# ZhicengShi/mclSTExp

Measured on AMD Instinct MI355X. Metric: training spots/sec (= steps/sec x global batch) at batch 128/GPU, 224px patches, 1000 genes, higher is better.
Workload: dtype bf16; 1 GPU; BASELINE configs[1]: train step, batch 128/GPU, 224x224 patches, 1000 genes, densenet121 image encoder; global_batch=128, parallelism=dp1, backbone_dtype=bf16, infonce=fused, infonce_effective=exact (fused from 1024 pairs), hip_graphs=True, optimizer=Adam(lr=1e-4, wd=1e-3) incl. 2x(65536,G) tables

## Files before the change

### include/mclstexp_hip.h

```cpp
#ifndef MCLSTEXP_HIP_H
#define MCLSTEXP_HIP_H

#include <stddef.h>
#include <stdint.h>

#ifdef __cplusplus
extern "C" {
#endif

#define MCL_ABI_VERSION 13

#define MCL_OK 0
#define MCL_EINVAL (-1)
#define MCL_EUNSUPPORTED (-2)
#define MCL_EWORKSPACE (-3)

typedef void* mcl_stream_t;

int mcl_abi_version(void);
const char* mcl_error_string(int code);

#define MCL_EPI_GELU 1
#define MCL_EPI_GELU_BWD 2
#define MCL_EPI_ACCUM 4
// ... 211 lines not shown
int mcl_dense_bn1_fix(const void* x, int64_t ldx, void* gbuf, int64_t ldg, int64_t S, int32_t c0, int32_t nc,
                      const float* mean, const float* rstd, const float* kacc, mcl_stream_t stream);
int mcl_conv1x1_wrw_det(const void* dz, int64_t ldz, const void* a, int64_t lda, const float* gamma, const float* beta,
                        const float* mean, const float* rstd, float* workspace, float* dW, int32_t accumulate_w,
                        int64_t S, int32_t M, int32_t N, mcl_stream_t stream);

int64_t mcl_dense_conv3x3_bwd_workspace_floats(int64_t S);
int mcl_dense_conv3x3_bwd(const void* dy, int64_t lddy, int64_t S, int32_t H, int32_t W, const void* W2, const void* z,
                          const float* gamma, const float* beta, const float* mean, const float* rstd, float* workspace,
                          float* dgamma, float* dbeta, int32_t accumulate_params, void* g2, void* dz, mcl_stream_t stream);
int mcl_dense_conv3x3_bwd_fix(const void* dy, int64_t lddy, int64_t S, int32_t H, int32_t W, const void* W2, const void* z,
                              const float* gamma, const float* beta, const float* mean, const float* rstd, float* workspace,
                              float* dgamma, float* dbeta, int32_t accumulate_params, void* g2, void* dz, const void* xfix,
                              int64_t ldxf, const float* fmean, const float* frstd, const float* fk, void* dyc,
                              mcl_stream_t stream);

int mcl_avgpool2_nhwc_bf16(const void* x, void* y, int32_t N, int32_t H, int32_t W, int32_t C, int32_t backward,
                           mcl_stream_t stream);
int mcl_maxpool3s2_nhwc_bf16_fwd(const void* x, void* y, void* idx, int32_t N, int32_t H, int32_t W, int32_t C,
                                 mcl_stream_t stream);
int mcl_maxpool3s2_nhwc_bf16_bwd(const void* idx, const void* dy, void* dx, int32_t N, int32_t H, int32_t W, int32_t C,
                                 mcl_stream_t stream);
int mcl_maxpool3s2_nhwc_bf16_bwd_ld(const void* idx, const void* dy, int64_t lddy, void* dx, int32_t N, int32_t H, int32_t W,
                                    int32_t C, mcl_stream_t stream);

int mcl_bn_act_avgpool_fwd(const void* x, int64_t ldx, int32_t N, int32_t H, int32_t W, int32_t C, const float* gamma,
                           const float* beta, const float* mean, const float* rstd, void* y, int64_t ldy,
                           mcl_stream_t stream);
int mcl_bn_act_avgpool_bwd(const void* dp, int64_t lddp, const void* x, int64_t ldx, int32_t N, int32_t H, int32_t W,
                           int32_t C, const float* gamma, const float* beta, const float* mean, const float* rstd,
// ... 214 lines not shown
```

### mclstexp_amd/_lib.py

```python
from __future__ import annotations

import ctypes as C
import os
from typing import Optional

import torch

_HERE = os.path.dirname(os.path.abspath(__file__))
LIB_PATH = os.environ.get("MCL_LIB_PATH") or os.path.join(_HERE, "libmclstexp_hip.so")
ABI_VERSION = 13

_lib: Optional[C.CDLL] = None

c_f = C.c_float
c_d = C.c_double
c_i = C.c_int32
c_l = C.c_int64
c_p = C.c_void_p


class GemmArgs(C.Structure):
    _fields_ = [
        ("struct_size", C.c_uint32),
        ("M", c_i), ("N", c_i), ("K", c_i), ("batch", c_i),
# ... 117 lines not shown
    "mcl_bn_workspace_floats": [c_l, c_i, c_i],
    "mcl_bn_stats": [c_p, c_l, c_l, c_i, c_i, c_p, c_l, c_p, c_f, c_p, c_p, c_p, c_p],
    "mcl_bn_act_fwd": [c_p, c_l, c_l, c_i, c_i, c_p, c_p, c_p, c_p, c_i, c_p, c_l, c_p],
    "mcl_bn_act_bwd": [c_p, c_l, c_p, c_l, c_l, c_i, c_i, c_p, c_p, c_p, c_p, c_i, c_p, c_p, c_p, c_i, c_p, c_l, c_i, c_p],
    "mcl_dense_conv1x1_workspace_floats": [c_l],
    "mcl_dense_conv1x1_fwd": [c_p, c_l, c_l, c_i, c_p, c_p, c_p, c_p, c_p, c_p, c_l, c_p, c_f, c_p, c_p, c_p, c_p],
    "mcl_dense_conv3x3_workspace_floats": [c_l],
    "mcl_dense_bn1_bwd_workspace_floats": [c_l, c_i],
    "mcl_dense_conv3x3_bwd_workspace_floats": [c_l],
    "mcl_avgpool2_nhwc_bf16": [c_p, c_p, c_i, c_i, c_i, c_i, c_i, c_p],
    "mcl_maxpool3s2_nhwc_bf16_fwd": [c_p, c_p, c_p, c_i, c_i, c_i, c_i, c_p],
    "mcl_maxpool3s2_nhwc_bf16_bwd": [c_p, c_p, c_p, c_i, c_i, c_i, c_i, c_p],
    "mcl_dense_conv3x3_bwd": [c_p, c_l, c_l, c_i, c_i, c_p, c_p, c_p, c_p, c_p, c_p, c_p, c_p, c_p, c_i, c_p, c_p, c_p],
    "mcl_dense_conv3x3_bwd_fix": [c_p, c_l, c_l, c_i, c_i, c_p, c_p, c_p, c_p, c_p, c_p, c_p, c_p, c_p, c_i, c_p, c_p, c_p,
                                  c_l, c_p, c_p, c_p, c_p, c_p],
    "mcl_dense_bn1_bwd": [c_p, c_p, c_i, c_p, c_l, c_l, c_p, c_p, c_p, c_p, c_p, c_p, c_p, c_i, c_p, c_l, c_p],
    "mcl_dense_conv3x3_wrw_workspace_floats": [c_l],
    "mcl_dense_conv3x3_wrw_det": [c_p, c_l, c_p, c_l, c_i, c_i, c_p, c_p, c_p, c_p, c_p, c_p, c_i, c_p],
    "mcl_wrw_workspace_floats": [c_l, c_i, c_i],
    "mcl_dense_bn1_wrw": [c_p, c_p, c_i, c_p, c_l, c_l, c_p, c_p, c_p, c_p, c_p, c_p, c_i, c_p, c_p, c_i, c_p, c_p],
    "mcl_dense_bn1_dx_window": [c_p, c_p, c_i, c_i, c_i, c_p, c_l, c_l, c_p, c_p, c_p, c_p, c_p, c_p, c_l, c_p],
    "mcl_dense_bn1_dx_pair": [c_p, c_p, c_i, c_p, c_p, c_p, c_p, c_p, c_p, c_p, c_p, c_i, c_p, c_l, c_l, c_p, c_p, c_p, c_l, c_p],
    "mcl_dense_bn1_dx": [c_p, c_p, c_i, c_p, c_l, c_l, c_p, c_p, c_p, c_p, c_p, c_p, c_l, c_p],
    "mcl_dense_bn1_dx_sums": [c_p, c_p, c_i, c_p, c_l, c_l, c_p, c_p, c_p, c_p, c_p, c_p, c_p, c_i, c_p, c_i, c_p, c_l, c_p],
    "mcl_dense_bn1_fix": [c_p, c_l, c_p, c_l, c_l, c_i, c_i, c_p, c_p, c_p, c_p],
    "mcl_conv1x1_wrw_det": [c_p, c_l, c_p, c_l, c_p, c_p, c_p, c_p, c_p, c_p, c_i, c_l, c_i, c_i, c_p],
    "mcl_dense_conv3x3_fwd": [c_p, c_l, c_i, c_i, c_p, c_p, c_p, c_p, c_p, c_p, c_l, c_p, c_f, c_p, c_p, c_p, c_p],
    "mcl_accum_into_f32": [c_p, c_p, c_l, c_i, c_p],
    "mcl_adam_step": [c_p, c_p, c_p, c_p, c_l, c_d, c_d, c_d, c_d, c_d, c_d, c_d, c_p],
    "mcl_adam_table_step": [c_p, c_p, c_p, c_i, c_i, c_p, c_p, c_l, c_d, c_d, c_d, c_d, c_d, c_d, c_d, c_p],
# ... 161 lines not shown
```

### mclstexp_amd/csrc/dense_bwd.hip

```cpp
#include "common.h"
#include <stdlib.h>

namespace {

constexpr int TN = 128, TK = 128;

template <int MODE, int TMv>
__global__ __launch_bounds__(256, (TMv == 64 && MODE != 2 ? 3 : 2)) void bn1_bwd_kernel(const bf16_t* __restrict__ dz, const bf16_t* __restrict__ W1,
                                                         int K , int ldw ,
                                                         const bf16_t* __restrict__ x, long long ldx, long long S,
                                                         const float* __restrict__ gamma,
                                                         const float* __restrict__ beta,
                                                         const float* __restrict__ mean,
                                                         const float* __restrict__ rstd,
                                                         const float* __restrict__ coef ,
                                                         bf16_t* gbuf, long long ldg,
                                                         float2* __restrict__ partial , int nrt) {
  __shared__ __attribute__((aligned(16))) unsigned char lds[TK * 256 + TMv * 256 + 2048];
  const int tid = threadIdx.x, lane = tid & 63, wave = tid >> 6;
  const int h = lane >> 5, l31 = lane & 31;
  const int wm = wave >> 1, wn = wave & 1;
  const int n0 = blockIdx.y * TN;
  unsigned char* wt = lds;
  unsigned char* dzt = lds + TK * 256;
// ... 838 lines not shown
    const unsigned gw[4] = {gv.x, gv.y, gv.z, gv.w}, zw[4] = {zv.x, zv.y, zv.z, zv.w};
    unsigned o[4];
#pragma unroll
    for (int u = 0; u < 4; ++u) {
      const float g_lo = __uint_as_float(gw[u] << 16), g_hi = __uint_as_float(gw[u] & 0xFFFF0000u);
      const float z_lo = __uint_as_float(zw[u] << 16), z_hi = __uint_as_float(zw[u] & 0xFFFF0000u);
      const float d_lo = sc[2 * u] * (g_lo - c1[2 * u] - (z_lo - mu[2 * u]) * rs[2 * u] * c2[2 * u]);
      const float d_hi = sc[2 * u + 1] * (g_hi - c1[2 * u + 1] - (z_hi - mu[2 * u + 1]) * rs[2 * u + 1] * c2[2 * u + 1]);
      const f32x2 pv = {d_lo, d_hi};
      o[u] = __builtin_bit_cast(unsigned, __builtin_convertvector(pv, bf16x2_t));
    }
    *reinterpret_cast<uint4*>(dz + q * 8) = make_uint4(o[0], o[1], o[2], o[3]);
  }
}

}

extern "C" int64_t mcl_dense_bn1_bwd_workspace_floats(int64_t S, int32_t C) {
  if (S <= 0 || C <= 0) return -1;
  return ((S + 63) / 64) * 2 * (int64_t)C + 2 * (int64_t)C;
}

extern "C" int mcl_dense_bn1_bwd(const void* dz, const void* W1, int32_t C, const void* x, int64_t ldx, int64_t S,
                                 const float* gamma, const float* beta, const float* mean, const float* rstd,
                                 float* workspace, float* dgamma, float* dbeta, int32_t accumulate_params, void* gbuf,
                                 int64_t ldg, mcl_stream_t stream) {
  MCL_CLEAR_ERROR();
  if (!dz || !W1 || !x || !gamma || !beta || !mean || !rstd || !workspace || !dgamma || !dbeta || !gbuf || S <= 0 || C <= 0)
    return MCL_EINVAL;
  if ((C % 8) || (ldx % 8) || (ldg % 8) || (reinterpret_cast<uintptr_t>(dz) & 15u) ||
// ... 129 lines not shown
                     (const bf16_t*)x, (long long)ldx, (long long)S, mean, rstd, (bf16_t*)gbuf, (long long)ldg, nrt);
  MCL_CHECK_LAUNCH();
  return MCL_OK;
}

extern "C" int64_t mcl_dense_conv3x3_bwd_workspace_floats(int64_t S) {
  if (S <= 0) return -1;
  const int64_t flat = (S + T3B - 1) / T3B, rows = S / 32 + 8;
  return (flat > rows ? flat : rows) * 2 * (int64_t)C3I + 2 * (int64_t)C3I;
}

namespace {
int conv3x3_bwd_impl(const void* dy, int64_t lddy, int64_t S, int32_t H, int32_t W, const void* W2, const void* z,
                     const float* gamma, const float* beta, const float* mean, const float* rstd, float* workspace,
                     float* dgamma, float* dbeta, int32_t accumulate_params, void* g2, void* dz, const void* xfix,
                     int64_t ldxf, const float* fmean, const float* frstd, const float* fk, void* dyc, mcl_stream_t stream) {
  MCL_CLEAR_ERROR();
  if (!dy || !W2 || !z || !gamma || !beta || !mean || !rstd || !workspace || !dgamma || !dbeta || !g2 || !dz || S <= 0 ||
      H <= 0 || W <= 0)
    return MCL_EINVAL;
  if ((S % ((int64_t)H * W)) || S > 0x7fff0000LL || W > 150 || (lddy % 8) || lddy < C3O ||
      (reinterpret_cast<uintptr_t>(dy) & 15u) || (reinterpret_cast<uintptr_t>(z) & 15u) ||
      (reinterpret_cast<uintptr_t>(g2) & 15u) || (reinterpret_cast<uintptr_t>(dz) & 15u))
    return MCL_EUNSUPPORTED;
  if (xfix != nullptr) {
    if (!fmean || !frstd || !fk || !dyc) return MCL_EINVAL;
    if (bwd_rows_applicable(S, H, W) || (ldxf % 8) || (reinterpret_cast<uintptr_t>(xfix) & 15u) ||
        (reinterpret_cast<uintptr_t>(dyc) & 15u))
      return MCL_EUNSUPPORTED;
  }
  hipStream_t st = mcl_stream(stream);
  float2* part = reinterpret_cast<float2*>(workspace);
// ... 10 lines not shown
                       (const bf16_t*)dy, (long long)lddy, p.nimg, H, W, (const bf16_t*)W2, (const bf16_t*)z, gamma, beta,
                       mean, rstd, (bf16_t*)g2, part, p.nsu, p.rc, p.nchunk, p.nstrip);
    hipLaunchKernelGGL(bn1_bwd_finalize_kernel, dim3(C3I), dim3(256), 0, st, (const float2*)part, p.nsu, C3I,
                       (long long)S, dgamma, dbeta, coef, accumulate_params);
  } else {
    const int ntile = (int)((S + T3B - 1) / T3B);
    coef = workspace + (int64_t)ntile * 2 * C3I;
    const size_t lds_bytes = (size_t)T3B * 256 + (size_t)(T3B + 2 * W + 2) * 64 + 64;
    const int gcap = S >= 50000 ? 512 : 768;
    hipLaunchKernelGGL(conv3x3_bwd_kernel, dim3(ntile < gcap ? ntile : gcap), dim3(256), lds_bytes, st, (const bf16_t*)dy,
                       (long long)lddy, (long long)S, H, W, (const bf16_t*)W2, (const bf16_t*)z, gamma, beta, mean, rstd,
                       (bf16_t*)g2, part, ntile, (const bf16_t*)xfix, (long long)ldxf, fmean, frstd, fk, (bf16_t*)dyc);
    hipLaunchKernelGGL(bn1_bwd_finalize_kernel, dim3(C3I), dim3(256), 0, st, (const float2*)part, ntile, C3I,
                       (long long)S, dgamma, dbeta, coef, accumulate_params);
  }
  const long long n_chunks = S * (C3I / 8);
  long long blocks = (n_chunks + 255) / 256;
  if (blocks > 2048) blocks = 2048;
  hipLaunchKernelGGL(bn2_dz_kernel, dim3((unsigned)blocks), dim3(256), 0, st, (const bf16_t*)g2, (const bf16_t*)z,
                     n_chunks, gamma, mean, rstd, (const float*)coef, (bf16_t*)dz);
  MCL_CHECK_LAUNCH();
  return MCL_OK;
}
}

extern "C" int mcl_dense_conv3x3_bwd(const void* dy, int64_t lddy, int64_t S, int32_t H, int32_t W, const void* W2,
                                     const void* z, const float* gamma, const float* beta, const float* mean,
                                     const float* rstd, float* workspace, float* dgamma, float* dbeta,
                                     int32_t accumulate_params, void* g2, void* dz, mcl_stream_t stream) {
  return conv3x3_bwd_impl(dy, lddy, S, H, W, W2, z, gamma, beta, mean, rstd, workspace, dgamma, dbeta, accumulate_params, g2,
                          dz, nullptr, 0, nullptr, nullptr, nullptr, nullptr, stream);
}

extern "C" int mcl_dense_conv3x3_bwd_fix(const void* dy, int64_t lddy, int64_t S, int32_t H, int32_t W, const void* W2,
                                         const void* z, const float* gamma, const float* beta, const float* mean,
                                         const float* rstd, float* workspace, float* dgamma, float* dbeta,
                                         int32_t accumulate_params, void* g2, void* dz, const void* xfix, int64_t ldxf,
                                         const float* fmean, const float* frstd, const float* fk, void* dyc,
                                         mcl_stream_t stream) {
  if (!xfix) return MCL_EINVAL;
  return conv3x3_bwd_impl(dy, lddy, S, H, W, W2, z, gamma, beta, mean, rstd, workspace, dgamma, dbeta, accumulate_params, g2,
                          dz, xfix, ldxf, fmean, frstd, fk, dyc, stream);
}
```

### mclstexp_amd/densenet_fused.py

```python
from __future__ import annotations

import contextlib
import os
from typing import List, NamedTuple, Optional, Tuple

import torch
import torch.nn.functional as F
from torch import nn

from . import _lib
from ._lib import check

Tensor = torch.Tensor
CL = torch.channels_last
_ws_cache = {}

_fallbacks: dict = {}


def fallback_counts() -> dict:
    return dict(_fallbacks)


def reset_fallbacks() -> None:
# ... 334 lines not shown
                 gbuf: Tensor, window=None) -> None:
    px, S, C, ldx = _rows(x)
    pg, S2, C2, ldg = _rows(gbuf)
    assert (S2, C2) == (S, C)
    L = _lib.lib()
    if window is None:
        check(L.mcl_dense_bn1_dx(dz.data_ptr(), w16.data_ptr(), C, px, ldx, S, g1.data_ptr(), b1.data_ptr(),
                                 mean.data_ptr(), rstd.data_ptr(), coef.data_ptr(), pg, ldg, _stream()), "mcl_dense_bn1_dx")
    else:
        c0, nc = window
        check(L.mcl_dense_bn1_dx_window(dz.data_ptr(), w16.data_ptr(), C, c0, nc, px, ldx, S, g1.data_ptr(), b1.data_ptr(),
                                        mean.data_ptr(), rstd.data_ptr(), coef.data_ptr(), pg, ldg, _stream()),
              "mcl_dense_bn1_dx_window")


def dense_bn1_dx_pair(A, B, x: Tensor, mean: Tensor, rstd: Tensor, gbuf: Tensor) -> None:
    dzA, wA, gA, bA, cA = A
    dzB, wB, gB, bB, cB = B
    px, S, C, ldx = _rows(x)
    pg, S2, C2, ldg = _rows(gbuf)
    assert (S2, C2) == (S, C) and wA.shape[1] >= C and wB.shape[1] == C
    check(_lib.lib().mcl_dense_bn1_dx_pair(dzA.data_ptr(), wA.data_ptr(), wA.shape[1], gA.data_ptr(), bA.data_ptr(), cA.data_ptr(),
                                           dzB.data_ptr(), wB.data_ptr(), gB.data_ptr(), bB.data_ptr(), cB.data_ptr(), C, px, ldx, S,
                                           mean.data_ptr(), rstd.data_ptr(), pg, ldg, _stream()), "mcl_dense_bn1_dx_pair")




def _c3_flat_kernel(W: int) -> bool:
    return W < 17 or W > 150


def dense_conv3x3_bwd(dy: Tensor, w16: Tensor, z: Tensor, g2: Tensor, b2: Tensor, m2: Tensor, r2: Tensor,
                      into_param_grads: bool, fix=None) -> Tuple[Tensor, Optional[Tensor], Optional[Tensor], Optional[Tensor]]:
    B, C, H, W = z.shape
    pd, S, Co, lddy = _rows(dy)
    assert C == 128 and Co == 32 and S == B * H * W and z.is_contiguous(memory_format=CL)
    L = _lib.lib()
    ws = _ws(L.mcl_dense_conv3x3_bwd_workspace_floats(S), z.device)
    scratch = torch.empty_like(z, memory_format=CL)
    dz = torch.empty_like(z, memory_format=CL)
    if into_param_grads:
        dg, db = g2.grad, b2.grad
    else:
        dg = torch.empty(C, device=z.device, dtype=torch.float32)
        db = torch.empty(C, device=z.device, dtype=torch.float32)
    dyc = None
    if fix is not None:
        xf, fm, fr, fk = fix
        pxf, S2, C2, ldxf = _rows(xf)
        assert (S2, C2) == (S, 32) and fk.is_contiguous() and fk.numel() == 64
        dyc = torch.empty((B, 32, H, W), device=z.device, dtype=z.dtype, memory_format=CL)
        check(L.mcl_dense_conv3x3_bwd_fix(pd, lddy, S, H, W, w16.data_ptr(), z.data_ptr(), g2.data_ptr(), b2.data_ptr(),
                                          m2.data_ptr(), r2.data_ptr(), ws.data_ptr(), dg.data_ptr(), db.data_ptr(),
                                          int(into_param_grads), scratch.data_ptr(), dz.data_ptr(), pxf, ldxf,
                                          fm.data_ptr(), fr.data_ptr(), fk.data_ptr(), dyc.data_ptr(), _stream()),
              "mcl_dense_conv3x3_bwd_fix")
    else:
        check(L.mcl_dense_conv3x3_bwd(pd, lddy, S, H, W, w16.data_ptr(), z.data_ptr(), g2.data_ptr(), b2.data_ptr(),
                                      m2.data_ptr(), r2.data_ptr(), ws.data_ptr(), dg.data_ptr(), db.data_ptr(),
                                      int(into_param_grads), scratch.data_ptr(), dz.data_ptr(), _stream()),
              "mcl_dense_conv3x3_bwd")
# ... 337 lines not shown
        m2, v2, r2 = bn2_stats[l]
        ptrs += [g1.data_ptr(), b1.data_ptr(), packed.data_ptr() + 2 * offs[l], g2.data_ptr(), b2.data_ptr(), w2c.data_ptr(),
                 zs[l].data_ptr(), m2.data_ptr(), v2.data_ptr(), r2.data_ptr()]
    arr = (C.c_void_p * len(ptrs))(*ptrs)
    nbytes = Lb.mcl_dense_block_fwd_workspace_bytes(B, L)
    ws = _ws((nbytes + 255 + 3) // 4 + 64, dev)
    base = (ws.data_ptr() + 255) & ~255
    from . import ops as _ops
    err = _ops.block_seam_error_flag(dev)
    px, S, C_, ld = _rows(buf)
    if ld != Ct:
        raise RuntimeError("dense_block_fwd_persistent: the concat buffer must be dense channels-last")
    check(Lb.mcl_dense_block_fwd(px, B, H, W, Ct, C0, L, arr, eps1, eps2, stats.mean.data_ptr(), stats.var.data_ptr(),
                                 stats.rstd.data_ptr(), base, err.data_ptr(), SEAM_MAX_SPINS, _stamps_ptr(), _stream()), "mcl_dense_block_fwd")
    return zs


class _LayerPlan(NamedTuple):
    conv2: str
    conv1: str
    fix: str
    lanes: bool
    opens_pair: bool


def _plan_layer(l: int, cin: int, growth: int, B: int, H: int, W: int, fused1: bool, fused2: bool, w1_direct: bool,
                w2_direct: bool, kacc_live: bool, side_stream: bool, single_pass: bool, single_max_map: int,
                gram_min_pixels: int) -> _LayerPlan:
    conv2 = "own" if fused2 and w2_direct else "generic"
    if not fused1:
# ... 143 lines not shown
                _side_join(dev)
                stamp(f"bwd block {buf.shape[2]}x{buf.shape[3]} after join (main)")
            return (gbuf[:, :C0], None, *grads)
        kacc = None
        pair_a = None
        pair_cin = 0

        def flush_pair():
            nonlocal pair_a
            if pair_a is not None:
                dzA, wA, gA, bA, cA = pair_a
                dense_bn1_dx(dzA, wA, buf[:, :pair_cin], gA, bA, stats.mean[:pair_cin], stats.rstd[:pair_cin], cA,
                             gbuf[:, :pair_cin], window=(0, pair_cin - growth))
                pair_a = None

        def gram_dx(opens_pair, dz, w1c, g1, b1, cin, coef):
            nonlocal pair_a, pair_cin
            mine = (dz, w1c, g1, b1, coef)
            if pair_a is not None:
                dense_bn1_dx_pair(pair_a, mine, buf[:, :cin], stats.mean[:cin], stats.rstd[:cin], gbuf[:, :cin])
                pair_a = None
            elif opens_pair:
                dense_bn1_dx(dz, w1c, buf[:, :cin], g1, b1, stats.mean[:cin], stats.rstd[:cin], coef, gbuf[:, :cin],
                             window=(cin - growth, growth))
                pair_a, pair_cin = mine, cin
            else:
                dense_bn1_dx(dz, w1c, buf[:, :cin], g1, b1, stats.mean[:cin], stats.rstd[:cin], coef, gbuf[:, :cin])
        for l in range(L - 1, -1, -1):
            g1, b1, w1, g2, b2, w2 = params[6 * l: 6 * l + 6]
            a, z, a2 = saved[3 * l: 3 * l + 3]
            w1c, w2c = wcast[2 * l: 2 * l + 2]
            cin = C0 + l * growth
            c1 = cin + growth
            m2, v2, r2 = bn2_stats[l]
            x, gx, mean1, rstd1 = buf[:, :cin], gbuf[:, :cin], stats.mean[:cin], stats.rstd[:cin]
            dy_view = gbuf[:, cin:c1]
            d2 = _direct_all(g2, b2)
            d1 = _direct_all(g1, b1)
            fused1 = a.numel() == 0
            fused2 = a2.numel() == 0 and _fused_3x3_ok(z, w2c)
            plan = _plan_layer(l, cin, growth, B, H, W, fused1, fused2, fused1 and _bn1_wrw_ok(w1),
                               fused2 and _wrw3_direct_ok(w2, z, dy_view), kacc is not None, USE_SIDE_STREAM,
                               USE_BN1_SINGLE_PASS, BN1_SINGLE_PASS_MAX_MAP, FUSED_BN1_WRW_MIN_PIXELS)
            fold = None
            if plan.fix == "fold":
                fold = (buf[:, cin:c1], stats.mean[cin:c1], stats.rstd[cin:c1], kacc[cin:c1])
            elif plan.fix == "launch_32":
                dense_bn1_fix(buf, gbuf, cin, growth, stats.mean, stats.rstd, kacc)
            elif plan.fix == "launch_all":
                dense_bn1_fix(buf, gbuf, 0, c1, stats.mean, stats.rstd, kacc)
                kacc = None
            dw2 = None
            if plan.conv2 == "own":
                dz, dg2, db2, dyc = dense_conv3x3_bwd(dy_view, w2c, z, g2, b2, m2, r2, into_param_grads=d2, fix=fold)
            else:
                dyc = None
                if a2.numel() == 0:
                    a2 = torch.empty_like(z, memory_format=CL)
                    bn_act_fwd(z, g2, b2, m2, r2, True, a2)
                da2, dw2 = _conv_bwd(dy_view, a2, w2c, w2, 1, ctx.kept_cols.pop(l, None))
                dz = torch.empty_like(z, memory_format=CL)
                dg2, db2 = bn_act_bwd(dense_cl(da2), z, g2, b2, m2, r2, True, dz, False, into_param_grads=d2)
            dy_w = dyc if dyc is not None else dy_view
            if ctx.cap is not None:
                ctx.cap["dz"][l] = dz
                ctx.cap["dyc"][l] = dyc
            ev = _fork_event(dev) if plan.lanes else None
            if plan.conv1 != "gram":
                flush_pair()
            gw1 = None
            if plan.conv1 == "gram":
                dg1, db1, coef = dense_bn1_wrw(dz, w1c, x, g1, b1, mean1, rstd1, w1, into_param_grads=d1)
                gram_dx(plan.opens_pair, dz, w1c, g1, b1, cin, coef)
            elif plan.conv1 == "single":
                have_prev = kacc is not None
                if not have_prev:
                    kacc = torch.empty((buf.shape[1], 2), device=dev, dtype=torch.float32)
                dg1, db1 = dense_bn1_dx_sums(dz, w1c, x, g1, b1, mean1, rstd1, gx, kacc, have_prev, into_param_grads=d1)
            elif plan.conv1 == "two_pass":
                dg1, db1 = dense_bn1_bwd(dz, w1c, x, g1, b1, mean1, rstd1, gx, into_param_grads=d1)
            else:
                da, dw1 = _conv1x1_bwd(dz, a, w1c, w1)
                dg1, db1 = bn_act_bwd(da, x, g1, b1, mean1, rstd1, True, gx, True, into_param_grads=d1)
                gw1 = None if dw1 is None else _wgrad(w1, dw1)

            def weight_grads():
                if plan.conv2 == "own":
                    done = dense_conv3x3_wrw(dy_w, z, g2, b2, m2, r2, w2)
# ... 603 lines not shown
```

### mclstexp_amd/kernel_costs.py

```python
from __future__ import annotations


def _conv1x1_wrw_det(a):
    S, M, N = a[11], a[12], a[13]
    return 2 * S * (M + N) + 4 * M * N


def _conv1x1_wrw_det_flops(a):
    return 2 * a[11] * a[12] * a[13]


def _conv3x3_wrw_det(a):
    S = a[3]
    return 2 * S * (32 + 128) + 4 * 32 * 1152


def _conv3x3_flops_S3(a):
    return 2 * a[3] * 32 * 1152


def _bn1_bwd(a):
    C, S = a[2], a[5]
    return 2 * S * (128 + C) + 2 * S * (128 + 3 * C)

# ... 16 lines not shown
    return 2 * a[2] * (32 + 128 + 128)


def _conv3x3_flops_S2(a):
    return 2 * a[2] * 32 * 1152


def _conv3x3_bwd_fix(a):
    return _conv3x3_bwd(a) + 2 * a[2] * (32 + 32)


def _conv3x3_bwd_fix_strict(a):
    return _conv3x3_bwd_strict(a) + 2 * a[2] * (32 + 32)


def _conv1x1_fwd(a):
    S, K = a[2], a[3]
    return 2 * S * (K + 128)


def _conv1x1_fwd_flops(a):
    return 2 * a[2] * a[3] * 128


def _conv3x3_fwd(a):
    S = a[1]
    return 2 * S * (128 + 32)


def _conv3x3_flops_S1(a):
# ... 9 lines not shown
    return 2 * 2 * a[5] * 128 * a[2]


def _bn1_dx(a):
    C, S = a[2], a[5]
    return 2 * S * (128 + 3 * C)


def _bn1_dx_window(a):
    nc, S = a[4], a[7]
    return 2 * S * (128 + 3 * nc)


def _bn1_dx_window_flops(a):
    return 2 * a[7] * 128 * a[4]


def _bn1_dx_pair(a):
    C, S = a[11], a[14]
    return 2 * S * (2 * 128 + 3 * C)


def _bn1_dx_pair_flops(a):
    return 2 * 2 * a[14] * 128 * a[11]


def _bn1_dx_sums(a):
    C, S = a[2], a[5]
    return 2 * S * (128 + 3 * C)

# ... 47 lines not shown

def _e(kernels, b, strict=None, flops=_zero, bound=None, unit=None):
    return {"kernels": kernels, "bytes": b, "strict": strict or b, "flops": flops, "bound": bound, "unit": unit}


TABLE = {
    "mcl_conv1x1_wrw_det": _e("wrw_partial_kernel + wrw_merge_kernel", _conv1x1_wrw_det, flops=_conv1x1_wrw_det_flops),
    "mcl_dense_conv3x3_wrw_det": _e("conv3x3_wrw_rows_kernel (56x56, 28x28 maps) / conv3x3_wrw_ky_kernel + wrw_merge_kernel",
                                    _conv3x3_wrw_det, flops=_conv3x3_flops_S3,
                                    bound="mfma/lds"),
    "mcl_dense_bn1_wrw": _e("wrw_partial_kernel<Gram> + wrw_merge_kernel", _bn1_wrw, flops=_bn1_wrw_flops),
    "mcl_dense_bn1_dx": _e("bn1_bwd_kernel<1> (one layer) / bn1_dx_pair_kernel (two consecutive layers' passes as one: "
                           "mcl_dense_bn1_dx_pair, preceded by the 32-channel mcl_dense_bn1_dx_window)", _bn1_dx, flops=_bn1_flops),
    "mcl_dense_bn1_dx_window": _e("bn1_bwd_kernel<1> on a 32-channel window", _bn1_dx_window, flops=_bn1_dx_window_flops,
                                  unit="mcl_dense_bn1_dx"),
    "mcl_dense_bn1_dx_pair": _e("bn1_dx_pair_kernel", _bn1_dx_pair, flops=_bn1_dx_pair_flops, unit="mcl_dense_bn1_dx"),
    "mcl_dense_bn1_dx_sums": _e("bn1_bwd_kernel<2> (single pass: dx data term + previous layer's mean terms + sums) + "
                                "bn1_bwd_finalize_kernel", _bn1_dx_sums, flops=_bn1_flops),
    "mcl_dense_bn1_fix": _e("bn1_fix_kernel", _bn1_fix, bound="latency"),
    "mcl_dense_bn1_bwd": _e("bn1_bwd_kernel<0> + bn1_bwd_finalize_kernel + bn1_bwd_kernel<1>", _bn1_bwd, _bn1_bwd_strict,
                            flops=lambda a: 2 * _bn1_flops(a)),
    "mcl_dense_conv3x3_bwd": _e("conv3x3_bwd_rows_kernel (56x56, 28x28 maps) / conv3x3_bwd_kernel (14x14, 7x7; with the "
                                "folded bn1_fix as mcl_dense_conv3x3_bwd_fix) + bn1_bwd_finalize_kernel + bn2_dz_kernel",
                                _conv3x3_bwd, _conv3x3_bwd_strict, flops=_conv3x3_flops_S2, bound="mfma/lds"),
    "mcl_dense_conv3x3_bwd_fix": _e("conv3x3_bwd_kernel (folded bn1_fix) + bn1_bwd_finalize_kernel + bn2_dz_kernel",
                                    _conv3x3_bwd_fix, _conv3x3_bwd_fix_strict, flops=_conv3x3_flops_S2, bound="mfma/lds",
                                    unit="mcl_dense_conv3x3_bwd"),
    "mcl_dense_conv1x1_fwd": _e("conv1x1_fwd_kernel + tile_stats_finalize_kernel", _conv1x1_fwd, flops=_conv1x1_fwd_flops),
    "mcl_dense_conv3x3_fwd": _e("conv3x3_fwd_rows_kernel + sums_finalize_kernel (56x56, 28x28 maps) / conv3x3_fwd_kernel + "
                                "tile_stats_finalize_kernel", _conv3x3_fwd, flops=_conv3x3_flops_S1, bound="mfma/lds"),
    "mcl_adam_table_step_dev": _e("adam_table_kernel", _adam_table, bound="hbm"),
    "mcl_dense_block_fwd": _e("dense_block_fwd_kernel (a whole 7x7 dense block forward: one persistent launch, in-launch batch-statistics "
                              "seams) + zero_words_kernel", _block_fwd, flops=_block_fwd_flops, bound="latency"),
    "mcl_dense_block_bwd": _e("dense_block_bwd_kernel (the block's data-gradient chain: one persistent launch) + zero_words_kernel",
                              _block_bwd, flops=_block_bwd_flops, bound="latency"),
    "mcl_adam_table_lazy": _e("adam_table_lazy_kernel (catch-up of gathered rows / update of the rows with a gradient)",
                              _adam_table_lazy, bound="latency"),
    "mcl_adam_step_dev": _e("adam_kernel", _adam, bound="hbm"),
    "mcl_adam_step_dev_shadow": _e("adam_kernel<shadow> (update + bf16 shadow of the parameters)", _adam_shadow, bound="hbm"),
}
```

Measured before the change: 12270 spots/s.

## Fuse windowed dz·W1 product into bn2 dz kernel and apply via stash

For DenseNet layers that open a bn1-dx pair, the bn2 dz kernel now also computes the 32-channel window product dz·W1 with MFMA while dz is still in LDS, and writes it to an fp32 stash. A new lightweight apply kernel then adds the bn1 backward term from that stash into gbuf, so the separate windowed bn1_dx kernel no longer has to re-read dz. The aim is to avoid one full pass over dz and its GEMM, at the cost of an extra S×32 fp32 stash write and read plus a stash allocation per layer. The path can be turned off with MCL_WINDOW_STASH=0.

Result: no change. 12320 spots/s (median of 6 runs) (+0.5%).

```diff
diff --git a/include/mclstexp_hip.h b/include/mclstexp_hip.h
--- a/include/mclstexp_hip.h
+++ b/include/mclstexp_hip.h
@@ -249,6 +249,13 @@
                               float* dgamma, float* dbeta, int32_t accumulate_params, void* g2, void* dz, const void* xfix,
                               int64_t ldxf, const float* fmean, const float* frstd, const float* fk, void* dyc,
                               mcl_stream_t stream);
+int mcl_dense_conv3x3_bwd_win(const void* dy, int64_t lddy, int64_t S, int32_t H, int32_t W, const void* W2, const void* z,
+                              const float* gamma, const float* beta, const float* mean, const float* rstd, float* workspace,
+                              float* dgamma, float* dbeta, int32_t accumulate_params, void* g2, void* dz, const void* W1win,
+                              int64_t ldw, int32_t nc, float* da_stash, mcl_stream_t stream);
+int mcl_dense_bn1_dx_window_apply(const float* da_stash, int32_t c0, int32_t nc, const void* x, int64_t ldx, int64_t S,
+                                  const float* gamma, const float* beta, const float* mean, const float* rstd,
+                                  const float* coef, void* gbuf, int64_t ldg, mcl_stream_t stream);
 
 int mcl_avgpool2_nhwc_bf16(const void* x, void* y, int32_t N, int32_t H, int32_t W, int32_t C, int32_t backward,
                            mcl_stream_t stream);
diff --git a/mclstexp_amd/_lib.py b/mclstexp_amd/_lib.py
--- a/mclstexp_amd/_lib.py
+++ b/mclstexp_amd/_lib.py
@@ -155,6 +155,9 @@
     "mcl_dense_conv3x3_bwd": [c_p, c_l, c_l, c_i, c_i, c_p, c_p, c_p, c_p, c_p, c_p, c_p, c_p, c_p, c_i, c_p, c_p, c_p],
     "mcl_dense_conv3x3_bwd_fix": [c_p, c_l, c_l, c_i, c_i, c_p, c_p, c_p, c_p, c_p, c_p, c_p, c_p, c_p, c_i, c_p, c_p, c_p,
                                   c_l, c_p, c_p, c_p, c_p, c_p],
+    "mcl_dense_conv3x3_bwd_win": [c_p, c_l, c_l, c_i, c_i, c_p, c_p, c_p, c_p, c_p, c_p, c_p, c_p, c_p, c_i, c_p, c_p, c_p,
+                                  c_l, c_i, c_p, c_p],
+    "mcl_dense_bn1_dx_window_apply": [c_p, c_i, c_i, c_p, c_l, c_l, c_p, c_p, c_p, c_p, c_p, c_p, c_l, c_p],
     "mcl_dense_bn1_bwd": [c_p, c_p, c_i, c_p, c_l, c_l, c_p, c_p, c_p, c_p, c_p, c_p, c_p, c_i, c_p, c_l, c_p],
     "mcl_dense_conv3x3_wrw_workspace_floats": [c_l],
     "mcl_dense_conv3x3_wrw_det": [c_p, c_l, c_p, c_l, c_i, c_i, c_p, c_p, c_p, c_p, c_p, c_p, c_i, c_p],
diff --git a/mclstexp_amd/csrc/dense_bwd.hip b/mclstexp_amd/csrc/dense_bwd.hip
--- a/mclstexp_amd/csrc/dense_bwd.hip
+++ b/mclstexp_amd/csrc/dense_bwd.hip
@@ -876,6 +876,154 @@
   }
 }
 
+constexpr int WIN_TM = 128;
+__global__ __launch_bounds__(256, 2) void bn2_dz_win_kernel(const bf16_t* __restrict__ g2, const bf16_t* __restrict__ z, long long S,
+                                                            const float* __restrict__ gamma, const float* __restrict__ mean,
+                                                            const float* __restrict__ rstd, const float* __restrict__ coef,
+                                                            bf16_t* __restrict__ dz, const bf16_t* __restrict__ W1w, int ldw,
+                                                            float* __restrict__ stash, int ntile) {
+  __shared__ __attribute__((aligned(16))) unsigned char dzt[WIN_TM * 256];
+  const int tid = threadIdx.x, lane = tid & 63, wave = tid >> 6;
+  const int h = lane >> 5, l31 = lane & 31;
+  const int cc = tid & 15, rr = tid >> 4;
+  constexpr int NL = WIN_TM / 16;
+  u32x4 gr[NL], zr[NL];
+  auto issue_loads = [&](int t) {
+    const long long row0 = (long long)t * WIN_TM;
+#pragma unroll
+    for (int i = 0; i < NL; ++i) {
+      long long rg = row0 + rr + 16 * i;
+      rg = rg < S ? rg : S - 1;
+      gr[i] = *reinterpret_cast<const u32x4*>(g2 + rg * 128 + cc * 8);
+      zr[i] = *reinterpret_cast<const u32x4*>(z + rg * 128 + cc * 8);
+    }
+  };
+  issue_loads(blockIdx.x);
+  {
+    u32x4 wv[2];
+#pragma unroll
+    for (int i = 0; i < 2; ++i) {
+      const int idx = tid + 256 * i;
+      wv[i] = *reinterpret_cast<const u32x4*>(W1w + (long long)(idx >> 2) * ldw + (idx & 3) * 8);
+    }
+#pragma unroll
+    for (int i = 0; i < 2; ++i) *reinterpret_cast<u32x4*>(dzt + (tid + 256 * i) * 16) = wv[i];
+  }
+  __syncthreads();
+  bf16x8 fb[8];
+#pragma unroll
+  for (int ks = 0; ks < 8; ++ks)
+#pragma unroll
+    for (int e = 0; e < 8; ++e)
+      fb[ks][e] = (short)*reinterpret_cast<const bf16_t*>(dzt + (16 * ks + 8 * h + e) * 64 + l31 * 2);
+  float mu[8], rs[8], sc[8], c1[8], c2[8];
+#pragma unroll
+  for (int i = 0; i < 8; ++i) {
+    const int c = cc * 8 + i;
+    mu[i] = mean[c];
+    rs[i] = rstd[c];
+    sc[i] = gamma[c] * rs[i];
+    c1[i] = coef[2 * c];
+    c2[i] = coef[2 * c + 1];
+  }
+
+  for (int t = blockIdx.x; t < ntile; t += gridDim.x) {
+    const long long row0 = (long long)t * WIN_TM;
+    __syncthreads();
+#pragma unroll
+    for (int i = 0; i < NL; ++i) {
+      unsigned o[4];
+#pragma unroll
+      for (int u = 0; u < 4; ++u) {
+        const float g_lo = __uint_as_float(gr[i][u] << 16), g_hi = __uint_as_float(gr[i][u] & 0xFFFF0000u);
+        const float z_lo = __uint_as_float(zr[i][u] << 16), z_hi = __uint_as_float(zr[i][u] & 0xFFFF0000u);
+        const float d_lo = sc[2 * u] * (g_lo - c1[2 * u] - (z_lo - mu[2 * u]) * rs[2 * u] * c2[2 * u]);
+        const float d_hi = sc[2 * u + 1] * (g_hi - c1[2 * u + 1] - (z_hi - mu[2 * u + 1]) * rs[2 * u + 1] * c2[2 * u + 1]);
+        const f32x2 pv = {d_lo, d_hi};
+        o[u] = __builtin_bit_cast(unsigned, __builtin_convertvector(pv, bf16x2_t));
+      }
+      const u32x4 ov = {o[0], o[1], o[2], o[3]};
+      const int r = rr + 16 * i;
+      if (row0 + r < S) *reinterpret_cast<u32x4*>(dz + (row0 + r) * 128 + cc * 8) = ov;
+      *reinterpret_cast<u32x4*>(dzt + r * 256 + ((cc ^ (r & 15)) << 4)) = ov;
+    }
+    if (t + (int)gridDim.x < ntile) issue_loads(t + gridDim.x);
+    __syncthreads();
+    f32x16 acc;
+#pragma unroll
+    for (int r = 0; r < 16; ++r) acc[r] = 0.0f;
+    const int ra = wave * 32 + l31;
+#pragma unroll
+    for (int ks = 0; ks < 8; ++ks) {
+      const bf16x8 fa = *reinterpret_cast<const bf16x8*>(dzt + ra * 256 + (((2 * ks + h) ^ (ra & 15)) << 4));
+      acc = __builtin_amdgcn_mfma_f32_32x32x16_bf16(fa, fb[ks], acc, 0, 0, 0);
+    }
+#pragma unroll
+    for (int r = 0; r < 16; ++r) {
+      const long long rg = row0 + wave * 32 + (r & 3) + 8 * (r >> 2) + 4 * h;
+      if (rg < S) stash[rg * 32 + l31] = acc[r];
+    }
+  }
+}
+
+__global__ __launch_bounds__(256) void bn1_win_apply_kernel(const float* __restrict__ stash, const bf16_t* __restrict__ x,
+                                                            long long ldx, long long S, const float* __restrict__ gamma,
+                                                            const float* __restrict__ beta, const float* __restrict__ mean,
+                                                            const float* __restrict__ rstd, const float* __restrict__ coef,
+                                                            bf16_t* __restrict__ gbuf, long long ldg) {
+  const long long n = S * 4;
+  const long long i0 = (long long)blockIdx.x * 256 + threadIdx.x, istride = (long long)gridDim.x * 256;
+  const int c = (threadIdx.x & 3) * 8;
+  u32x4 xa, ga, xb, gb;
+  f32x4 a0, a1, b0, b1;
+  auto issue_loads = [&](long long i) {
+    const long long ra = i >> 2;
+    const long long rb = i + istride < n ? (i + istride) >> 2 : ra;
+    a0 = *reinterpret_cast<const f32x4*>(stash + ra * 32 + c);
+    a1 = *reinterpret_cast<const f32x4*>(stash + ra * 32 + c + 4);
+    b0 = *reinterpret_cast<const f32x4*>(stash + rb * 32 + c);
+    b1 = *reinterpret_cast<const f32x4*>(stash + rb * 32 + c + 4);
+    xa = *reinterpret_cast<const u32x4*>(x + ra * ldx + c);
+    xb = *reinterpret_cast<const u32x4*>(x + rb * ldx + c);
+    ga = *reinterpret_cast<const u32x4*>(gbuf + ra * ldg + c);
+    gb = *reinterpret_cast<const u32x4*>(gbuf + rb * ldg + c);
+  };
+  issue_loads(i0 < n ? i0 : n - 4 + (threadIdx.x & 3));
+  float sc[8], sh[8], ka[8], kb[8];
+#pragma unroll
+  for (int e = 0; e < 8; ++e) {
+    const float mu = mean[c + e], rs = rstd[c + e];
+    sc[e] = gamma[c + e] * rs;
+    sh[e] = fmaf(-mu, sc[e], beta[c + e]);
+    const float k1 = coef[2 * (c + e)], k2 = coef[2 * (c + e) + 1];
+    ka[e] = -sc[e] * k2 * rs;
+    kb[e] = fmaf(-ka[e], mu, -sc[e] * k1);
+  }
+  auto apply = [&](const f32x4& d0, const f32x4& d1, const u32x4& xv, const u32x4& gv) {
+    const float da[8] = {d0[0], d0[1], d0[2], d0[3], d1[0], d1[1], d1[2], d1[3]};
+    u32x4 ov;
+#pragma unroll
+    for (int u = 0; u < 4; ++u) {
+      const float x_lo = __uint_as_float(xv[u] << 16), x_hi = __uint_as_float(xv[u] & 0xFFFF0000u);
+      const float gi_lo = fmaf(x_lo, sc[2 * u], sh[2 * u]) > 0.0f ? da[2 * u] : 0.0f;
+      const float gi_hi = fmaf(x_hi, sc[2 * u + 1], sh[2 * u + 1]) > 0.0f ? da[2 * u + 1] : 0.0f;
+      const unsigned dl = f2bf(fmaf(sc[2 * u], gi_lo, fmaf(ka[2 * u], x_lo, kb[2 * u])));
+      const unsigned dh = f2bf(fmaf(sc[2 * u + 1], gi_hi, fmaf(ka[2 * u + 1], x_hi, kb[2 * u + 1])));
+      const float lo = __uint_as_float(gv[u] << 16) + __uint_as_float(dl << 16);
+      const float hi = __uint_as_float(gv[u] & 0xFFFF0000u) + __uint_as_float(dh << 16);
+      const f32x2 pv = {lo, hi};
+      ov[u] = __builtin_bit_cast(unsigned, __builtin_convertvector(pv, bf16x2_t));
+    }
+    return ov;
+  };
+  for (long long i = i0; i < n; i += 2 * istride) {
+    if (i != i0) issue_loads(i);
+    const u32x4 oa = apply(a0, a1, xa, ga), ob = apply(b0, b1, xb, gb);
+    *reinterpret_cast<u32x4*>(gbuf + (i >> 2) * ldg + c) = oa;
+    if (i + istride < n) *reinterpret_cast<u32x4*>(gbuf + ((i + istride) >> 2) * ldg + c) = ob;
+  }
+}
+
 }
 
 extern "C" int64_t mcl_dense_bn1_bwd_workspace_floats(int64_t S, int32_t C) {
@@ -1035,8 +1183,15 @@
 int conv3x3_bwd_impl(const void* dy, int64_t lddy, int64_t S, int32_t H, int32_t W, const void* W2, const void* z,
                      const float* gamma, const float* beta, const float* mean, const float* rstd, float* workspace,
                      float* dgamma, float* dbeta, int32_t accumulate_params, void* g2, void* dz, const void* xfix,
-                     int64_t ldxf, const float* fmean, const float* frstd, const float* fk, void* dyc, mcl_stream_t stream) {
+                     int64_t ldxf, const float* fmean, const float* frstd, const float* fk, void* dyc, mcl_stream_t stream,
+                     bool win = false, const void* W1win = nullptr, int64_t ldw = 0, int32_t nc = 0, float* da_stash = nullptr) {
   MCL_CLEAR_ERROR();
+  if (win) {
+    if (!W1win || !da_stash || ldw <= 0 || nc <= 0) return MCL_EINVAL;
+    if (nc != 32 || ldw < nc || (ldw % 8) || (reinterpret_cast<uintptr_t>(W1win) & 15u) ||
+        (reinterpret_cast<uintptr_t>(da_stash) & 15u) || xfix != nullptr)
+      return MCL_EUNSUPPORTED;
+  }
   if (!dy || !W2 || !z || !gamma || !beta || !mean || !rstd || !workspace || !dgamma || !dbeta || !g2 || !dz || S <= 0 ||
       H <= 0 || W <= 0)
     return MCL_EINVAL;
@@ -1077,11 +1232,18 @@
     hipLaunchKernelGGL(bn1_bwd_finalize_kernel, dim3(C3I), dim3(256), 0, st, (const float2*)part, ntile, C3I,
                        (long long)S, dgamma, dbeta, coef, accumulate_params);
   }
-  const long long n_chunks = S * (C3I / 8);
-  long long blocks = (n_chunks + 255) / 256;
-  if (blocks > 2048) blocks = 2048;
-  hipLaunchKernelGGL(bn2_dz_kernel, dim3((unsigned)blocks), dim3(256), 0, st, (const bf16_t*)g2, (const bf16_t*)z,
-                     n_chunks, gamma, mean, rstd, (const float*)coef, (bf16_t*)dz);
+  if (win) {
+    const int ntile = (int)((S + WIN_TM - 1) / WIN_TM), rounds = (ntile + 511) / 512;
+    hipLaunchKernelGGL(bn2_dz_win_kernel, dim3((unsigned)((ntile + rounds - 1) / rounds)), dim3(256), 0, st, (const bf16_t*)g2,
+                       (const bf16_t*)z, (long long)S, gamma, mean, rstd, (const float*)coef, (bf16_t*)dz, (const bf16_t*)W1win,
+                       (int)ldw, da_stash, ntile);
+  } else {
+    const long long n_chunks = S * (C3I / 8);
+    long long blocks = (n_chunks + 255) / 256;
+    if (blocks > 2048) blocks = 2048;
+    hipLaunchKernelGGL(bn2_dz_kernel, dim3((unsigned)blocks), dim3(256), 0, st, (const bf16_t*)g2, (const bf16_t*)z,
+                       n_chunks, gamma, mean, rstd, (const float*)coef, (bf16_t*)dz);
+  }
   MCL_CHECK_LAUNCH();
   return MCL_OK;
 }
@@ -1093,6 +1255,33 @@
                                      int32_t accumulate_params, void* g2, void* dz, mcl_stream_t stream) {
   return conv3x3_bwd_impl(dy, lddy, S, H, W, W2, z, gamma, beta, mean, rstd, workspace, dgamma, dbeta, accumulate_params, g2,
                           dz, nullptr, 0, nullptr, nullptr, nullptr, nullptr, stream);
+}
+
+extern "C" int mcl_dense_conv3x3_bwd_win(const void* dy, int64_t lddy, int64_t S, int32_t H, int32_t W, const void* W2,
+                                         const void* z, const float* gamma, const float* beta, const float* mean,
+                                         const float* rstd, float* workspace, float* dgamma, float* dbeta,
+                                         int32_t accumulate_params, void* g2, void* dz, const void* W1win, int64_t ldw,
+                                         int32_t nc, float* da_stash, mcl_stream_t stream) {
+  return conv3x3_bwd_impl(dy, lddy, S, H, W, W2, z, gamma, beta, mean, rstd, workspace, dgamma, dbeta, accumulate_params, g2,
+                          dz, nullptr, 0, nullptr, nullptr, nullptr, nullptr, stream, true, W1win, ldw, nc, da_stash);
+}
+
+extern "C" int mcl_dense_bn1_dx_window_apply(const float* da_stash, int32_t c0, int32_t nc, const void* x, int64_t ldx, int64_t S,
+                                             const float* gamma, const float* beta, const float* mean, const float* rstd,
+                                             const float* coef, void* gbuf, int64_t ldg, mcl_stream_t stream) {
+  MCL_CLEAR_ERROR();
+  if (!da_stash || !x || !gamma || !beta || !mean || !rstd || !coef || !gbuf || S <= 0 || c0 < 0 || nc <= 0 || (c0 % 8))
+    return MCL_EINVAL;
+  if (nc != 32 || (ldx % 8) || (ldg % 8) || ldx < nc || ldg < nc || (reinterpret_cast<uintptr_t>(da_stash) & 15u) ||
+      (reinterpret_cast<uintptr_t>(x) & 15u) || (reinterpret_cast<uintptr_t>(gbuf) & 15u))
+    return MCL_EUNSUPPORTED;
+  long long nb = (S * 4 + 511) / 512;
+  if (nb > 2048) nb = 2048;
+  hipLaunchKernelGGL(bn1_win_apply_kernel, dim3((unsigned)nb), dim3(256), 0, mcl_stream(stream), da_stash,
+                     (const bf16_t*)x + c0, (long long)ldx, (long long)S, gamma + c0, beta + c0, mean + c0, rstd + c0,
+                     coef + 2 * c0, (bf16_t*)gbuf + c0, (long long)ldg);
+  MCL_CHECK_LAUNCH();
+  return MCL_OK;
 }
 
 extern "C" int mcl_dense_conv3x3_bwd_fix(const void* dy, int64_t lddy, int64_t S, int32_t H, int32_t W, const void* W2,
diff --git a/mclstexp_amd/densenet_fused.py b/mclstexp_amd/densenet_fused.py
--- a/mclstexp_amd/densenet_fused.py
+++ b/mclstexp_amd/densenet_fused.py
@@ -372,6 +372,16 @@
               "mcl_dense_bn1_dx_window")
 
 
+def dense_bn1_dx_window_apply(stash: Tensor, c0: int, x: Tensor, g1: Tensor, b1: Tensor, mean: Tensor, rstd: Tensor, coef: Tensor,
+                              gbuf: Tensor) -> None:
+    px, S, C, ldx = _rows(x)
+    pg, S2, C2, ldg = _rows(gbuf)
+    assert (S2, C2) == (S, C) and stash.shape == (S, 32) and stash.is_contiguous()
+    check(_lib.lib().mcl_dense_bn1_dx_window_apply(stash.data_ptr(), c0, 32, px, ldx, S, g1.data_ptr(), b1.data_ptr(),
+                                                   mean.data_ptr(), rstd.data_ptr(), coef.data_ptr(), pg, ldg, _stream()),
+          "mcl_dense_bn1_dx_window_apply")
+
+
 def dense_bn1_dx_pair(A, B, x: Tensor, mean: Tensor, rstd: Tensor, gbuf: Tensor) -> None:
     dzA, wA, gA, bA, cA = A
     dzB, wB, gB, bB, cB = B
@@ -390,7 +400,7 @@
 
 
 def dense_conv3x3_bwd(dy: Tensor, w16: Tensor, z: Tensor, g2: Tensor, b2: Tensor, m2: Tensor, r2: Tensor,
-                      into_param_grads: bool, fix=None) -> Tuple[Tensor, Optional[Tensor], Optional[Tensor], Optional[Tensor]]:
+                      into_param_grads: bool, fix=None, window=None):
     B, C, H, W = z.shape
     pd, S, Co, lddy = _rows(dy)
     assert C == 128 and Co == 32 and S == B * H * W and z.is_contiguous(memory_format=CL)
@@ -404,6 +414,18 @@
         dg = torch.empty(C, device=z.device, dtype=torch.float32)
         db = torch.empty(C, device=z.device, dtype=torch.float32)
     dyc = None
+    if window is not None:
+        assert fix is None
+        w1c, c0 = window
+        ldw = w1c.shape[1]
+        assert w1c.shape[0] == 128 and w1c.numel() == 128 * ldw and w1c.is_contiguous() and 0 <= c0 <= ldw - 32
+        stash = torch.empty((S, 32), device=z.device, dtype=torch.float32)
+        check(L.mcl_dense_conv3x3_bwd_win(pd, lddy, S, H, W, w16.data_ptr(), z.data_ptr(), g2.data_ptr(), b2.data_ptr(),
+                                          m2.data_ptr(), r2.data_ptr(), ws.data_ptr(), dg.data_ptr(), db.data_ptr(),
+                                          int(into_param_grads), scratch.data_ptr(), dz.data_ptr(),
+                                          w1c.data_ptr() + c0 * w1c.element_size(), ldw, 32, stash.data_ptr(), _stream()),
+              "mcl_dense_conv3x3_bwd_win")
+        return (dz, None, None, None, stash) if into_param_grads else (dz, dg, db, None, stash)
     if fix is not None:
         xf, fm, fr, fk = fix
         pxf, S2, C2, ldxf = _rows(xf)
@@ -771,6 +793,9 @@
     check(Lb.mcl_dense_block_fwd(px, B, H, W, Ct, C0, L, arr, eps1, eps2, stats.mean.data_ptr(), stats.var.data_ptr(),
                                  stats.rstd.data_ptr(), base, err.data_ptr(), SEAM_MAX_SPINS, _stamps_ptr(), _stream()), "mcl_dense_block_fwd")
     return zs
+
+
+USE_WINDOW_STASH = os.environ.get("MCL_WINDOW_STASH", "1") != "0"
 
 
 class _LayerPlan(NamedTuple):
@@ -944,15 +969,19 @@
                              gbuf[:, :pair_cin], window=(0, pair_cin - growth))
                 pair_a = None
 
-        def gram_dx(opens_pair, dz, w1c, g1, b1, cin, coef):
+        def gram_dx(opens_pair, dz, w1c, g1, b1, cin, coef, stash=None):
             nonlocal pair_a, pair_cin
             mine = (dz, w1c, g1, b1, coef)
             if pair_a is not None:
                 dense_bn1_dx_pair(pair_a, mine, buf[:, :cin], stats.mean[:cin], stats.rstd[:cin], gbuf[:, :cin])
                 pair_a = None
             elif opens_pair:
-                dense_bn1_dx(dz, w1c, buf[:, :cin], g1, b1, stats.mean[:cin], stats.rstd[:cin], coef, gbuf[:, :cin],
-                             window=(cin - growth, growth))
+                if stash is not None:
+                    dense_bn1_dx_window_apply(stash, cin - growth, buf[:, :cin], g1, b1, stats.mean[:cin], stats.rstd[:cin],
+                                              coef, gbuf[:, :cin])
+                else:
+                    dense_bn1_dx(dz, w1c, buf[:, :cin], g1, b1, stats.mean[:cin], stats.rstd[:cin], coef, gbuf[:, :cin],
+                                 window=(cin - growth, growth))
                 pair_a, pair_cin = mine, cin
             else:
                 dense_bn1_dx(dz, w1c, buf[:, :cin], g1, b1, stats.mean[:cin], stats.rstd[:cin], coef, gbuf[:, :cin])
@@ -981,8 +1010,14 @@
                 dense_bn1_fix(buf, gbuf, 0, c1, stats.mean, stats.rstd, kacc)
                 kacc = None
             dw2 = None
+            stash = None
             if plan.conv2 == "own":
-                dz, dg2, db2, dyc = dense_conv3x3_bwd(dy_view, w2c, z, g2, b2, m2, r2, into_param_grads=d2, fix=fold)
+                if (USE_WINDOW_STASH and plan.opens_pair and pair_a is None and fold is None and w1c.is_contiguous()
+                        and w1c.shape[0] == 128 and w1c.shape[1] == cin):
+                    dz, dg2, db2, dyc, stash = dense_conv3x3_bwd(dy_view, w2c, z, g2, b2, m2, r2, into_param_grads=d2,
+                                                                 window=(w1c, cin - growth))
+                else:
+                    dz, dg2, db2, dyc = dense_conv3x3_bwd(dy_view, w2c, z, g2, b2, m2, r2, into_param_grads=d2, fix=fold)
             else:
                 dyc = None
                 if a2.numel() == 0:
@@ -1001,7 +1036,8 @@
             gw1 = None
             if plan.conv1 == "gram":
                 dg1, db1, coef = dense_bn1_wrw(dz, w1c, x, g1, b1, mean1, rstd1, w1, into_param_grads=d1)
-                gram_dx(plan.opens_pair, dz, w1c, g1, b1, cin, coef)
+                gram_dx(plan.opens_pair, dz, w1c, g1, b1, cin, coef, stash)
+                stash = None
             elif plan.conv1 == "single":
                 have_prev = kacc is not None
                 if not have_prev:
diff --git a/mclstexp_amd/kernel_costs.py b/mclstexp_amd/kernel_costs.py
--- a/mclstexp_amd/kernel_costs.py
+++ b/mclstexp_amd/kernel_costs.py
@@ -54,6 +54,18 @@
     return _conv3x3_bwd_strict(a) + 2 * a[2] * (32 + 32)
 
 
+def _conv3x3_bwd_win(a):
+    return _conv3x3_bwd(a) + 4 * a[2] * 32
+
+
+def _conv3x3_bwd_win_strict(a):
+    return _conv3x3_bwd_strict(a) + 4 * a[2] * 32
+
+
+def _conv3x3_bwd_win_flops(a):
+    return _conv3x3_flops_S2(a) + 2 * a[2] * 128 * 32
+
+
 def _conv1x1_fwd(a):
     S, K = a[2], a[3]
     return 2 * S * (K + 128)
@@ -93,6 +105,11 @@
 
 def _bn1_dx_window_flops(a):
     return 2 * a[7] * 128 * a[4]
+
+
+def _bn1_dx_window_apply(a):
+    nc, S = a[2], a[5]
+    return S * nc * (4 + 3 * 2)
 
 
 def _bn1_dx_pair(a):
@@ -170,6 +187,8 @@
                            "mcl_dense_bn1_dx_pair, preceded by the 32-channel mcl_dense_bn1_dx_window)", _bn1_dx, flops=_bn1_flops),
     "mcl_dense_bn1_dx_window": _e("bn1_bwd_kernel<1> on a 32-channel window", _bn1_dx_window, flops=_bn1_dx_window_flops,
                                   unit="mcl_dense_bn1_dx"),
+    "mcl_dense_bn1_dx_window_apply": _e("bn1_win_apply_kernel (the windowed term from the product mcl_dense_conv3x3_bwd_win left)",
+                                        _bn1_dx_window_apply, unit="mcl_dense_bn1_dx"),
     "mcl_dense_bn1_dx_pair": _e("bn1_dx_pair_kernel", _bn1_dx_pair, flops=_bn1_dx_pair_flops, unit="mcl_dense_bn1_dx"),
     "mcl_dense_bn1_dx_sums": _e("bn1_bwd_kernel<2> (single pass: dx data term + previous layer's mean terms + sums) + "
                                 "bn1_bwd_finalize_kernel", _bn1_dx_sums, flops=_bn1_flops),
@@ -181,6 +200,10 @@
                                 _conv3x3_bwd, _conv3x3_bwd_strict, flops=_conv3x3_flops_S2, bound="mfma/lds"),
     "mcl_dense_conv3x3_bwd_fix": _e("conv3x3_bwd_kernel (folded bn1_fix) + bn1_bwd_finalize_kernel + bn2_dz_kernel",
                                     _conv3x3_bwd_fix, _conv3x3_bwd_fix_strict, flops=_conv3x3_flops_S2, bound="mfma/lds",
+                                    unit="mcl_dense_conv3x3_bwd"),
+    "mcl_dense_conv3x3_bwd_win": _e("conv3x3_bwd_rows_kernel / conv3x3_bwd_kernel + bn1_bwd_finalize_kernel + bn2_dz_win_kernel "
+                                    "(dz and the 32-channel window product dz W1 of the layer that opens a pair)",
+                                    _conv3x3_bwd_win, _conv3x3_bwd_win_strict, flops=_conv3x3_bwd_win_flops, bound="mfma/lds",
                                     unit="mcl_dense_conv3x3_bwd"),
     "mcl_dense_conv1x1_fwd": _e("conv1x1_fwd_kernel + tile_stats_finalize_kernel", _conv1x1_fwd, flops=_conv1x1_fwd_flops),
     "mcl_dense_conv3x3_fwd": _e("conv3x3_fwd_rows_kernel + sums_finalize_kernel (56x56, 28x28 maps) / conv3x3_fwd_kernel + "
```
